# pentalpha/sickle

Hardware: AMD Instinct MI355X
Metric: reads/sec trimmed (+ Gbases/sec), 150 bp SE Sanger q20 l20, inputs resident in HBM (higher is better)
Workload: dtype u8; 1 GPU; sickle se, 10000000 synthetic 150 bp Sanger reads per GPU, q=20 l=20 (BASELINE configs[1]); mode=resident, reads_per_gpu=10000000, reads_in_job=10000000, read_len=150, stride=152, kernel=sk_scan_tile_staged_kernel

## Files before the change

### sickle_amd/csrc/sk_kernels.hip

```cpp

#include "sk_kernel_common.h"

#ifndef SK_WIDE_QUIET
#define SK_WIDE_QUIET 1
#endif
#define SK_STAGE_MIN 5
#define SK_STAGE_MAX 20
#ifndef SK_CUT_STORE_AUX
#define SK_CUT_STORE_AUX 16
#endif


template <bool UNIFORM, bool HAS_SEQ, bool MFMA, int NBUF, int ABLATE, int SEG, int STAGE, bool RAG, bool SORT = false, int WIDE = 0, int WSTAGE = 0>
__device__ __forceinline__ void
sk_scan_tile_body(const uint8_t *__restrict__ qual, const uint8_t *__restrict__ seq,
                  const uint32_t *__restrict__ lengths, sk_cut_dev *__restrict__ out,
                  unsigned long long *errword, const sk_scan_args &a, const sk_tile_dev *__restrict__ tiles,
                  const uint32_t *__restrict__ out_index, const uint64_t *__restrict__ offsets)
{
    static_assert(!SORT || (RAG && !UNIFORM && MFMA), "regrouped ragged batches: re-strided tiles, matrix path");
    static_assert(!WIDE || (RAG && UNIFORM && MFMA && !SORT), "medium reads: uniform batches, re-strided tiles, matrix path");
    static_assert(!WSTAGE || (WIDE && !HAS_SEQ), "the medium-read tiles' register stage: without -n");
    constexpr uint32_t ROWS = WIDE == 2 ? 16u : WIDE ? 32u : 64u;
    constexpr int RSHIFT = WIDE == 2 ? 4 : WIDE ? 5 : 6;
    static_assert(!RAG || (NBUF == 1 && !SEG && STAGE == 0 && ABLATE == 0), "re-strided tiles: one buffer, LDS-DMA");
    static_assert(!MFMA || UNIFORM || RAG, "the matrix path needs one window width per tile");
    constexpr bool MIXED = MFMA && !UNIFORM;
    static_assert(STAGE == 0 || (UNIFORM && !HAS_SEQ && NBUF == 1 && (SEG == 0 || SEG == 2)), "register staging: uniform tiles, one buffer");
    static_assert(!SEG || (UNIFORM && MFMA && NBUF == 1), "segmented batches run the uniform matrix path, one buffer");
    constexpr int LDS_BUFS = NBUF;
    constexpr bool SEQ_SHARES = HAS_SEQ && NBUF == 1;
    extern __shared__ __attribute__((aligned(16))) uint8_t lds[];
    const int lane = threadIdx.x & 63;
    const int rlane = WIDE == 2 ? (lane & 15) : WIDE ? (lane & 31) : lane;
    const int part = WIDE == 2 ? (lane >> 4) & 1 : 0;
    const int wave = __builtin_amdgcn_readfirstlane((int)(threadIdx.x >> 6));
    const int waves_per_block = blockDim.x >> 6;
    const uint32_t stride = a.stride;
    const uint32_t buf_bytes = (RAG || SEG) ? a.buf_bytes : 64u * stride + SK_TILE_SLACK;
    uint8_t *buf0 = lds + (size_t)wave * LDS_BUFS * buf_bytes;
    uint8_t *buf1 = LDS_BUFS > 1 ? buf0 + buf_bytes : buf0;

    const uint32_t xcd = SORT ? blockIdx.x & 7u : 0u;
    const unsigned long long *const slist = reinterpret_cast<const unsigned long long *>(tiles) + (size_t)xcd * a.n_tiles * 4u;
    const uint64_t *const perm = reinterpret_cast<const uint64_t *>(out_index) + (size_t)xcd * a.n_tiles * 64u;
    const uint64_t n_tiles = SORT ? (uint64_t)min(scalar_load(lengths + xcd), a.n_tiles) : SEG ? (uint64_t)a.n_tiles : (a.n_reads + ROWS - 1) >> RSHIFT;
    uint64_t wave_global = SORT ? (uint64_t)(blockIdx.x >> 3) : (uint64_t)blockIdx.x * waves_per_block + wave;
    const uint64_t wave_count = SORT ? (uint64_t)((gridDim.x - xcd + 7u) >> 3) : (uint64_t)gridDim.x * waves_per_block;
    if (a.tile_order == 1 && (wave_count & 7) == 0) {
        const uint64_t per = wave_count >> 3;
        wave_global = (wave_global & 7) * per + (wave_global >> 3);
    }

    const uint32_t min4 = splat((uint32_t)a.qmin), max4 = splat((uint32_t)a.qmax);
    const uint32_t hi4 = splat((uint32_t)(127 - a.qmax));
    const uint32_t cthr4 = splat((uint32_t)a.cthr);
    const int range = a.qmax - a.qmin;

    int Lu = 0, wu = 0;
    bool scan_u = false, three_blocks = false;
    sk_v4i bandA0 = {0, 0, 0, 0}, bandA1 = {0, 0, 0, 0}, bandA2 = {0, 0, 0, 0};
    sk_v16i negT;
    const int half = lane >> 5;
    constexpr bool TABLE = SEG != 0 || SORT;
    struct band3 {
        sk_v4i b0, b1, b2;
    };
    band3 band_next{{0, 0, 0, 0}, {0, 0, 0, 0}, {0, 0, 0, 0}};
    auto band_fetch = [&](int w) -> band3 {
        typedef const __attribute__((address_space(1))) sk_v4i *gv4;
        gv4 tb = (gv4)(uintptr_t)a.band_table + ((uint32_t)w * 3u * 64u + (uint32_t)lane);
        band3 b;
        b.b0 = tb[0];
        b.b1 = tb[64];
        b.b2 = (SEG == 2) ? b.b1 : tb[128];
        return b;
    };
    auto width_of = [](int len) -> int { return len / 10 ? len / 10 : len; };
    auto set_scalars = [&](int len) {
        const int w_old = wu;
        Lu = len;
        scan_u = Lu > 0 && Lu >= a.lthr;
        wu = width_of(Lu);
        three_blocks = MFMA && STAGE == 0 && (SEG == 2 ? false : SEG == 3 ? true : wu > 33);
        if (MFMA && (!TABLE || wu != w_old)) {
            const int T = a.craw * wu;
#pragma unroll
            for (int i = 0; i < 16; ++i) {
                int seed = -T;
                asm volatile("" : "+v"(seed));
                negT[i] = seed;
            }
        }
    };
    auto install_band = [&](const band3 &b) {
        bandA0 = b.b0;
        bandA1 = b.b1;
        bandA2 = b.b2;
    };
    auto set_length = [&](int len) {
        set_scalars(len);
        if (MFMA) {
            int ln = lane;
            if (MIXED) asm volatile("" : "+v"(ln));
            const int k0 = (ln >> 5) * 16;
            const int far = WIDE ? 32 * (wu / 32) : 32;
#pragma unroll
            for (int j = 0; j < 4; ++j) {
                bandA0[j] = (int)sk_band_dword(ln, wu, k0 + 4 * j);
                bandA1[j] = (int)sk_band_dword(ln, wu, k0 + 4 * j + far);
                bandA2[j] = (int)sk_band_dword(ln, wu, k0 + 4 * j + far + 32);
            }
        }
    };
    constexpr bool WRITE_THROUGH = STAGE != 0 && SEG == 0 && ABLATE != 3;
    if (!TABLE) set_length((int)a.read_len);

    const uint64_t batch_end = RAG ? rag_batch_end(offsets, lengths, a) : 0;
    auto fetch_desc = [&](uint64_t tt) -> sk_tile_dev {
        uint32_t at = (uint32_t)tt * (uint32_t)sizeof(sk_tile_dev);
        asm volatile("" : "+v"(at));
        return *reinterpret_cast<const sk_tile_dev *>(reinterpret_cast<const uint8_t *>(tiles) + at);
    };
    auto uniform_desc = [&](const sk_tile_dev &d) -> sk_tile_dev {
        sk_tile_dev u;
        u.byte_off = ((uint64_t)(uint32_t)__builtin_amdgcn_readfirstlane((int)(uint32_t)(d.byte_off >> 32)) << 32) |
                     (uint32_t)__builtin_amdgcn_readfirstlane((int)(uint32_t)d.byte_off);
        u.slot0 = (uint32_t)__builtin_amdgcn_readfirstlane((int)d.slot0);
        u.stride = (uint32_t)__builtin_amdgcn_readfirstlane((int)d.stride);
        const uint32_t rl = (uint32_t)__builtin_amdgcn_readfirstlane((int)((uint32_t)d.rows | ((uint32_t)d.read_len << 16)));
        u.rows = (uint16_t)rl;
        u.read_len = (uint16_t)(rl >> 16);
        u.reserved = 0;
        return u;
    };
    auto probe = [&](uint64_t tt, const sk_tile_dev *ahead = nullptr) -> sk_tile_view {
        sk_tile_view v;
        v.take = true;
        v.uni = false;
        v.rowoff = 0;
        if (SEG) {
            const sk_tile_dev d = ahead ? uniform_desc(*ahead) : tiles[tt];
            v.off = d.byte_off;
            v.ts = d.stride;
            v.rows = d.rows;
            v.bytes = v.rows * v.ts;
            v.len = (int)d.read_len;
            v.r = d.slot0;
        } else if (RAG && UNIFORM) {
            v.off = (tt << RSHIFT) * stride;
            v.rows = (uint32_t)min((uint64_t)ROWS, a.n_reads - (tt << RSHIFT));
            v.ts = rag_pitch<true>(a.read_len);
            v.bytes = (v.rows - 1u) * stride + a.read_len;
            v.len = (int)a.read_len;
            v.r = (tt << RSHIFT) + rlane;
        } else if (SORT) {
        } else if (RAG) {
            const sk_rag_tile g = rag_probe(tt, lane, offsets, lengths, a);
            v.off = g.start;
            v.bytes = g.span;
            v.rows = (uint32_t)min((uint64_t)64, a.n_reads - (tt << 6));
            v.ts = rag_pitch<false>((uint32_t)g.lmax);
            v.len = g.len;
            v.rowoff = g.rowoff;
            v.r = (tt << 6) + lane;
            v.take = rag_tile_fits(g, buf_bytes);
            v.uni = v.rows == 64u && __builtin_amdgcn_ballot_w64(g.len != g.lmax) == 0;
        } else {
            v.off = (tt << 6) * stride;
            v.rows = (uint32_t)min((uint64_t)64, a.n_reads - (tt << 6));
            v.ts = stride;
            v.bytes = v.rows * stride;
            v.r = (tt << 6) + lane;
            v.len = UNIFORM ? (int)a.read_len : (v.r < a.n_reads ? (int)min(lengths[v.r], stride) : 0);
        }
        return v;
    };

    struct sort_raw {
        sk_v4u d0, d1;
        uint64_t e;
    };
    auto sort_issue = [&](uint64_t tt) -> sort_raw {
        sort_raw q;
        uint32_t at = (uint32_t)tt * 32u;
        asm volatile("" : "+v"(at));
        const uint8_t *dp = reinterpret_cast<const uint8_t *>(slist) + at;
        q.d0 = *reinterpret_cast<const sk_v4u *>(dp);
        q.d1 = *reinterpret_cast<const sk_v4u *>(dp + 16);
        q.e = perm[tt * 64u + (uint32_t)lane];
        return q;
    };
    auto first = [](uint32_t x) -> uint32_t { return (uint32_t)__builtin_amdgcn_readfirstlane((int)x); };
    int sort_lmax = 0, sort_lmin = 0, sort_w = 0;
    int next_lmax = 0, next_lmin = 0, next_w = 0;
    auto sort_finish = [&](const sort_raw &q) -> sk_tile_view {
        sk_tile_view v;
        const uint32_t d00 = first(q.d0[0]), d01 = first(q.d0[1]), d02 = first(q.d0[2]), d03 = first(q.d0[3]);
        const uint32_t d10 = first(q.d1[0]), d11 = first(q.d1[1]), d12 = first(q.d1[2]);
        const uint64_t widx = d00;
        v.rows = (d01 >> 16) & 0xffu;
        next_w = (int)(d01 >> 24);
        next_lmax = (int)(d12 & 0xffffu);
        next_lmin = (int)(d12 >> 16);
        v.off = ((uint64_t)d03 << 32) | d02;
        v.bytes = d11 ? 0xffffffffu : d10;
        v.rowoff = (uint32_t)lane < v.rows ? (uint32_t)q.e : 0u;
        v.len = (uint32_t)lane < v.rows ? (int)((uint32_t)(q.e >> 32) & 0xffffu) : 0;
        v.r = widx * SK_SORT_WINDOW + (uint32_t)(q.e >> 48);
        v.ts = rag_pitch<false>((uint32_t)next_lmax);
        v.take = true;
        v.uni = true;
        return v;
    };

    auto probe_index = [&](sk_tile_view &v) { v.r = (uint64_t)((uint32_t)v.r + min((uint32_t)lane, v.rows - 1u)); };
    const bool scatter = SEG && !a.slot_order;
    auto index_issue = [&](uint64_t slot) -> uint32_t {
        uint32_t idx;
        const uint32_t *src = out_index + slot;
        asm volatile("global_load_dword %0, %1, off" : "=v"(idx) : "v"(src) : "memory");
        return idx;
    };
    auto index_settle = [&](uint32_t &idx) { asm volatile("s_waitcnt vmcnt(0)" : "+v"(idx)::"memory"); };

    typedef uint32_t sk_v4u_a4 __attribute__((ext_vector_type(4), aligned(1)));
    constexpr int WOFF = WIDE ? (WSTAGE ? WSTAGE : 32) : 0;
    uint32_t wso[WOFF ? WOFF : 1];
    sk_v4u wst[WSTAGE ? WSTAGE : 1];
    const uint32_t wpieces = WIDE ? (ROWS * (rag_pitch<true>(a.read_len) / 16u) + 63u) >> 6 : 0u;
    if (WIDE) {
        const uint32_t cpr = rag_pitch<true>(a.read_len) / 16u, qd = 64u / cpr, rd = 64u % cpr;
        const uint32_t lim = (ROWS - 1u) * stride + a.read_len - 1u;
        uint32_t rr = (uint32_t)lane / cpr, cc = (uint32_t)lane % cpr;
#pragma unroll
        for (int p = 0; p < WOFF; ++p) {
            wso[p] = min(__umul24(rr, stride) + 16u * cc, lim);
            cc += rd;
            rr += qd;
            if (cc >= cpr) {
                cc -= cpr;
                ++rr;
            }
        }
    }

    auto rag_dma = [&](const uint8_t *base, uint8_t *dst, const sk_tile_view &v) {
        constexpr uint32_t GRAN = 16u;
        const uint32_t cpr = v.ts / GRAN;
        const uint32_t qd = 64u / cpr, rd = 64u % cpr;
        uint32_t rr = (uint32_t)lane / cpr, cc = (uint32_t)lane % cpr;
        const uint8_t *src = base + v.off;
        const uint32_t lim = (v.bytes ? v.bytes : 1u) - 1u;
// ... 1 lines not shown
        if (WIDE && !WSTAGE && all_safe && v.rows == ROWS && wpieces <= (uint32_t)WOFF) {
#pragma unroll
            for (int p = 0; p < WOFF; ++p)
                if ((uint32_t)p < wpieces) dma_piece<true, false>(src + wso[p], dst + (uint32_t)p * (64u * GRAN));
            return;
        }
        auto piece = [&](uint32_t p, uint32_t ro, uint32_t cc_p) {
            const uint32_t so = min(ro + GRAN * cc_p, lim);
            const bool inside = all_safe || v.off + so + GRAN <= batch_end;
            if (__builtin_expect(all_safe || __builtin_amdgcn_ballot_w64(!inside) == 0, 1)) {
                dma_piece<true, SORT>(src + so, dst + p * (64u * GRAN));
            } else {
                if (inside) {
                    dma_piece<true, SORT>(src + so, dst + p * (64u * GRAN));
                } else {
                    for (uint32_t j = 0; j < GRAN && v.off + so + j < batch_end; ++j)
                        dst[p * (64u * GRAN) + (uint32_t)lane * GRAN + j] = src[so + j];
                }
            }
        };
        auto advance = [&]() {
            cc += rd;
            rr += qd;
            if (cc >= cpr) {
                cc -= cpr;
                ++rr;
            }
        };
        if (SORT) {
            for (uint32_t p = 0; p < cpr; p += 4) {
                uint32_t ro[4], cq[4];
#pragma unroll
                for (int u = 0; u < 4; ++u) {
                    ro[u] = (uint32_t)__builtin_amdgcn_ds_bpermute((int)(min(rr, 63u) << 2), (int)v.rowoff);
                    cq[u] = cc;
                    advance();
                }
#pragma unroll
                for (int u = 0; u < 4; ++u)
                    if (p + (uint32_t)u < cpr) piece(p + (uint32_t)u, ro[u], cq[u]);
            }
        } else {
            const uint32_t pieces = WIDE == 2 ? (cpr + 3u) >> 2 : WIDE ? (cpr + 1u) >> 1 : cpr;
            for (uint32_t p = 0; p < pieces; ++p) {
                uint32_t ro;
                if (UNIFORM) ro = WIDE ? __umul24(rr, stride) : rr * stride;
                else if (v.uni) ro = rr * (uint32_t)__builtin_amdgcn_readfirstlane(v.len);
                else ro = (uint32_t)__builtin_amdgcn_ds_bpermute((int)(rr << 2), (int)v.rowoff);
                piece(p, ro, cc);
                advance();
            }
        }
    };
    auto load_tile = [&](const uint8_t *base, uint8_t *dst, const sk_tile_view &v) {
        if (RAG) rag_dma(base, dst, v);
        else tile_to_lds(base + v.off, dst, v.bytes, lane);
    };

    auto wstage_ok = [&](const sk_tile_view &v) -> bool { return WSTAGE && v.rows == ROWS && v.off + (uint64_t)v.bytes + 16u <= batch_end; };
    auto wstage_load = [&](const sk_tile_view &v) {
        const uint8_t *src = qual + v.off;
#pragma unroll
        for (int p = 0; p < WSTAGE; ++p) wst[p] = __builtin_nontemporal_load(reinterpret_cast<const sk_v4u_a4 *>(src + wso[p]));
    };
    auto wstage_write = [&]() {
#pragma unroll
        for (int p = 0; p < WSTAGE; ++p)
            if ((uint32_t)p < wpieces) *reinterpret_cast<sk_v4u *>(buf0 + (uint32_t)p * 1024u + (uint32_t)lane * 16u) = wst[p];
    };
    bool w_cur = false, w_nxt = false;

    sk_v4u stage[STAGE ? STAGE : 1];
    const uint32_t full_bytes = 64u * stride;
    auto stage_off = [&](int p, uint32_t bytes) -> uint32_t {
        const uint32_t off = (uint32_t)p * 1024u + (uint32_t)lane * 16u;
        return (SEG || p == STAGE - 1) ? min(off, bytes - 16u) : off;
    };

    const uint64_t SEG_CHUNK = SORT ? 1ull : 1ull << a.seg_chunk_shift;
    auto next_tile = [&](uint64_t tt) -> uint64_t {
        if (SEG || SORT) return ((tt + 1) & (SEG_CHUNK - 1)) != 0 ? tt + 1 : tt + 1 + (wave_count - 1) * SEG_CHUNK;
        return tt + wave_count;
    };
    uint64_t t = (SEG || SORT) ? wave_global * SEG_CHUNK : wave_global;
    if (t >= n_tiles) return;

    sk_tile_view cur = SORT ? sort_finish(sort_issue(t)) : probe(t), nxt = cur;
    if (TABLE) band_next = band_fetch(SORT ? next_w : width_of(cur.len));
    sort_raw raw{{0, 0, 0, 0}, {0, 0, 0, 0}, 0};
    if (SEG) probe_index(cur);
    bool cur_staged = STAGE && cur.rows == 64u;
    if (cur_staged) {
        const uint32_t cb = SEG ? cur.bytes : full_bytes;
#pragma unroll
        for (int p = 0; p < STAGE; ++p)
            stage[p] = __builtin_nontemporal_load(reinterpret_cast<const sk_v4u *>(qual + cur.off + stage_off(p, cb)));
    } else if (wstage_ok(cur)) {
        wstage_load(cur);
        w_cur = true;
    } else if (cur.take) {
        load_tile(qual, buf0, cur);
    }
    if (HAS_SEQ && !SEQ_SHARES) tile_to_lds(seq + cur.off, buf1, cur.bytes, lane);
    int parity = 0;
    constexpr bool PROBE_EARLY = NBUF == 2 || STAGE != 0 || ABLATE != 0 || SEG != 0;

    sk_tile_dev ahead{};
    if (SEG) ahead = fetch_desc(min(next_tile(t), n_tiles - 1));
    for (; t < n_tiles; t = next_tile(t)) {
        const uint64_t tn = next_tile(t);
        const bool more = tn < n_tiles;
        if (PROBE_EARLY && more) nxt = probe(tn, SEG ? &ahead : nullptr);
        const uint32_t ts = cur.ts;
        const uint64_t r = cur.r;
        const uint32_t cur_bytes = cur.bytes;
        if (SEG && cur.len != Lu) {
            if (width_of(cur.len) != wu) install_band(band_next);
            set_scalars(cur.len);
        }
        const uint32_t next_bytes = (PROBE_EARLY && more) ? nxt.bytes : 0u;
        const int next_pieces = (PROBE_EARLY && more) ? tile_pieces(next_bytes) : 0;
        const uint8_t *tile;

        const bool active = (uint32_t)rlane < cur.rows;
        const int Lv = UNIFORM ? 0 : cur.len;
        bool tile_u = false;
        if (MIXED && SORT) {
            sort_lmax = next_lmax;
            sort_lmin = next_lmin;
            sort_w = next_w;
            tile_u = sort_w > 0;
            if (tile_u && sort_w != wu) {
                install_band(band_next);
                set_scalars(sort_lmax);
            }
        } else if (MIXED) {
            const int l0 = __builtin_amdgcn_readfirstlane(cur.len);
            tile_u = cur.uni && l0 > 0 && l0 / 10 <= 65;
            if (tile_u && l0 != Lu) set_length(l0);
        }

        if (SORT) {
            tile = buf0;
            wait_vmcnt(0);
            if (more) raw = sort_issue(tn);
        } else if (SEQ_SHARES || RAG) {
            tile = buf0;
            if (WSTAGE && w_cur) wstage_write();
            else wait_vmcnt(0);
        } else if (HAS_SEQ) {
            tile = buf0;
            wait_vmcnt(tile_pieces(cur_bytes));
        } else if (STAGE) {
            tile = buf0;
            const bool next_staged = more && nxt.rows == 64u && ABLATE != 2;
            if (SEG) {
                if (cur_staged && next_staged) {
                    const uint8_t *nsrc = qual + nxt.off;
#pragma unroll
                    for (int p = 0; p < STAGE; ++p) {
                        *reinterpret_cast<sk_v4u *>(buf0 + stage_off(p, cur_bytes)) = stage[p];
                        stage[p] = __builtin_nontemporal_load(reinterpret_cast<const sk_v4u *>(nsrc + stage_off(p, next_bytes)));
                    }
                } else {
                    if (cur_staged) {
#pragma unroll
                        for (int p = 0; p < STAGE; ++p) *reinterpret_cast<sk_v4u *>(buf0 + stage_off(p, cur_bytes)) = stage[p];
                    } else {
                        wait_vmcnt(0);
                    }
                    if (next_staged) {
                        const uint8_t *nsrc = qual + nxt.off;
#pragma unroll
                        for (int p = 0; p < STAGE; ++p)
                            stage[p] = __builtin_nontemporal_load(reinterpret_cast<const sk_v4u *>(nsrc + stage_off(p, next_bytes)));
                    }
                }
            } else if (cur_staged && (ABLATE != 2 || t == wave_global)) {
                const uint8_t *nsrc = qual + (next_staged ? nxt.off : cur.off);
                const uint32_t keep = next_staged ? ~0u : 1023u;
#pragma unroll
                for (int p = 0; p < STAGE; ++p) {
                    const uint32_t off = stage_off(p, full_bytes);
                    *reinterpret_cast<sk_v4u *>(buf0 + off) = stage[p];
                    stage[p] = __builtin_nontemporal_load(reinterpret_cast<const sk_v4u *>(nsrc + (off & keep)));
                }
            } else if (!cur_staged) {
                wait_vmcnt(0);
            }
            cur_staged = next_staged;
        } else if (NBUF == 1 || ABLATE == 2) {
            tile = buf0;
            wait_vmcnt(0);
        } else {
            tile = parity ? buf1 : buf0;
            uint8_t *other = parity ? buf0 : buf1;
            if (more) tile_to_lds(qual + nxt.off, other, next_bytes, lane);
            wait_vmcnt(next_pieces);
            parity ^= 1;
        }
        if (!PROBE_EARLY && !SORT && more) nxt = probe(tn);
        if (WSTAGE) {
            w_nxt = more && wstage_ok(nxt);
            if (w_nxt) wstage_load(nxt);
        }
        if (SEG) ahead = fetch_desc(min(next_tile(tn), n_tiles - 1));
        if (SEG && more) probe_index(nxt);
        if (SEG && more && width_of(nxt.len) != wu) band_next = band_fetch(width_of(nxt.len));
        uint32_t oidx = 0;
        if (scatter) oidx = index_issue(r);
        if (RAG && !cur.take) {
            if (lane == 0) {
                atomicMax(errword + 1, (unsigned long long)a.scan_id);
                atomicMax(errword + 6, (unsigned long long)(a.scan_id & 0xffffffffull) << 32);
                atomicAdd(errword + 6, 1ull);
            }
            if (more && nxt.take) load_tile(qual, buf0, nxt);
            cur = nxt;
            continue;
        }
        const uint32_t *row = reinterpret_cast<const uint32_t *>(tile + (size_t)rlane * ts);
        if (ABLATE == 1) {
            const sk_cut_dev dummy{(int)row[0], (int)row[1]};
            asm volatile("s_waitcnt lgkmcnt(0)" ::: "memory");
            if (NBUF == 1 && more && (!STAGE || !cur_staged)) tile_to_lds(qual + nxt.off, buf0, next_bytes, lane);
            if (active) out[r] = dummy;
            cur = nxt;
            continue;
        }

        const bool scanned = UNIFORM ? (active && scan_u) : (active && Lv > 0 && Lv >= a.lthr);
        const int L = UNIFORM ? (scan_u ? Lu : 0) : (scanned ? Lv : 0);
        int w = L / 10;
        if (w == 0) w = L;
        const int nwin = (UNIFORM ? scan_u : scanned) ? L - w + 1 : 0;
// ... 281 lines not shown
                const sk_v2u s5 = __builtin_amdgcn_permlane32_swap(h5, h5, false, false), s3 = __builtin_amdgcn_permlane32_swap(h3, h3, false, false);
                h5 = min(s5[0], s5[1]);
                h3 = min(s3[0], s3[1]);
                if (WIDE == 2) {
                    h5 = min(h5, (uint32_t)__builtin_amdgcn_ds_bpermute((lane ^ 16) << 2, (int)h5));
                    h3 = min(h3, (uint32_t)__builtin_amdgcn_ds_bpermute((lane ^ 16) << 2, (int)h3));
                }
            }
            if (have5 && h5 != NONE) five = 4 * k5 + (int)(h5 >> 3);
            if (done && h3 != NONE) three = 4 * k3 + (int)(h3 >> 3);
        }

        if (__builtin_amdgcn_ballot_w64(bad)) {
            if (bad) {
                const int touched = done ? i1 + w : L;
                int p = INF;
                for (int k = 0; 4 * k < L; ++k) {
                    uint32_t f = keep_first(bad_flags(row[k], min4, hi4), L - 4 * k);
                    if (f) { p = 4 * k + (__builtin_ctz(f) >> 3); break; }
                }
                if (p < touched) report_error(errword, SEG ? (uint64_t)out_index[r] : r, p, (int)(int8_t)(tile[(size_t)rlane * ts + p]));
            }
        }

        if (HAS_SEQ) {
            asm volatile("s_waitcnt lgkmcnt(0)" ::: "memory");
            if (SEQ_SHARES) {
                load_tile(seq, buf0, cur);
                wait_vmcnt(0);
                if (scatter) index_settle(oidx);
            } else {
                if (more) tile_to_lds(qual + nxt.off, buf0, next_bytes, lane);
                wait_vmcnt(next_pieces);
            }
            const uint32_t *srow = reinterpret_cast<const uint32_t *>((SEQ_SHARES ? buf0 : buf1) + (size_t)rlane * ts);
            uint32_t nlo = NONE, anyN = 0;
            auto n_step = [&](uint32_t x, uint32_t rel) {
                const uint32_t y = (x | 0x20202020u) ^ 0x6e6e6e6eu;
                const uint32_t either = ~(((y & 0x7f7f7f7fu) + 0x7f7f7f7fu) | y) & H4;
                const uint32_t lower = either & (x << 2);
                nlo = min(nlo, __builtin_elementwise_add_sat(ffbl_or_none(lower), rel));
                anyN |= either ^ lower;
            };
            {
                int k = 0;
                if (UNIFORM || tile_u) {
                    const int full = (SORT ? min(Lfull, Lmax) : Lmax) >> 2;
                    const uint64_t *srow64 = reinterpret_cast<const uint64_t *>(srow);
                    constexpr int SHARE = WIDE == 2 ? 4 : WIDE ? 2 : 1;
                    for (k = 8 * (WIDE == 2 ? lane >> 4 : WIDE ? half : 0); k + 8 <= full; k += 8 * SHARE) {
                        uint64_t x[4];
#pragma unroll
                        for (int u = 0; u < 4; ++u) x[u] = srow64[(k >> 1) + u];
#pragma unroll
                        for (int u = 0; u < 4; ++u) {
                            n_step((uint32_t)x[u], 32u * (uint32_t)(k + 2 * u));
                            n_step((uint32_t)(x[u] >> 32), 32u * (uint32_t)(k + 2 * u + 1));
                        }
                    }
                    if (WIDE) k = full & ~7;
                }
                for (; 4 * k < Lmax; ++k) n_step(first_bytes(srow[k], L - 4 * k, 0u), 32u * (uint32_t)k);
                if (WIDE) {
                    const sk_v2u sn = __builtin_amdgcn_permlane32_swap(nlo, nlo, false, false), sa = __builtin_amdgcn_permlane32_swap(anyN, anyN, false, false);
                    nlo = min(sn[0], sn[1]);
                    anyN = sa[0] | sa[1];
                    if (WIDE == 2) {
                        nlo = min(nlo, (uint32_t)__builtin_amdgcn_ds_bpermute((lane ^ 16) << 2, (int)nlo));
                        anyN |= (uint32_t)__builtin_amdgcn_ds_bpermute((lane ^ 16) << 2, (int)anyN);
                    }
                }
            }
            if (nlo != NONE) three = (int)(nlo >> 3) - 1;
            else if (anyN) three = -2;
            asm volatile("s_waitcnt lgkmcnt(0)" ::: "memory");
            if (SORT && more) {
                nxt = sort_finish(raw);
                if (next_w != wu && next_w != 0) band_next = band_fetch(next_w);
            }
            if (more) {
                if (SEQ_SHARES) { if (nxt.take) load_tile(qual, buf0, nxt); }
                else tile_to_lds(seq + nxt.off, buf1, next_bytes, lane);
            }
        } else if (NBUF == 1 && ABLATE != 2 && (!STAGE || (more && !cur_staged))) {
            asm volatile("s_waitcnt lgkmcnt(0)" ::: "memory");
            if (scatter) index_settle(oidx);
            if (SORT && more) {
                nxt = sort_finish(raw);
                if (next_w != wu && next_w != 0) band_next = band_fetch(next_w);
            }
            if (more && nxt.take && !(WSTAGE && w_nxt)) load_tile(qual, buf0, nxt);
        }
        if (WSTAGE) w_cur = w_nxt;
#if SK_TAIL_PRIO
        __builtin_amdgcn_s_setprio(0);
#endif

        if (!scanned || !found5 || (three - five < a.lthr)) {
            five = -1;
            three = -1;
        }
        if (STAGE && scatter) index_settle(oidx);
        if constexpr (WRITE_THROUGH) {
            typedef int sk_v2i __attribute__((ext_vector_type(2)));
            const __amdgpu_buffer_rsrc_t cuts = __builtin_amdgcn_make_buffer_rsrc(out + (t << 6), 0, (int)(cur.rows * 8u), 0x00020000);
            if (active) __builtin_amdgcn_raw_buffer_store_b64(sk_v2i{five, three}, cuts, lane * 8, 0, SK_CUT_STORE_AUX);
        } else if (active && (!WIDE || lane < (int)ROWS)) {
            out[scatter ? (uint64_t)oidx : r] = sk_cut_dev{five, three};
        }
        asm volatile("s_waitcnt lgkmcnt(0)" ::: "memory");
        cur = nxt;
    }
}

template <bool UNIFORM, bool HAS_SEQ, bool MFMA = false, int NBUF = 2, int ABLATE = 0, int SEG = 0>
__global__ void __launch_bounds__(SK_TILE_THREADS, 2)
sk_scan_tile_kernel(const uint8_t *__restrict__ qual, const uint8_t *__restrict__ seq,
                    const uint32_t *__restrict__ lengths, sk_cut_dev *__restrict__ out,
                    unsigned long long *errword, sk_scan_args a, const sk_tile_dev *__restrict__ tiles = nullptr,
                    const uint32_t *__restrict__ out_index = nullptr)
{
    sk_scan_tile_body<UNIFORM, HAS_SEQ, MFMA, NBUF, ABLATE, SEG, 0, false>(qual, seq, lengths, out, errword, a, tiles, out_index, nullptr);
}

template <bool UNIFORM, bool HAS_SEQ, bool MFMA>
__global__ void __launch_bounds__(SK_TILE_THREADS, 2)
sk_scan_tile_any_kernel(const uint8_t *__restrict__ qual, const uint8_t *__restrict__ seq,
                        const uint64_t *__restrict__ offsets, const uint32_t *__restrict__ lengths,
                        sk_cut_dev *__restrict__ out, unsigned long long *errword, sk_scan_args a)
{
    if (!UNIFORM && a.sort_flags && scalar_load(a.sort_flags) != 0 && scalar_load(a.sort_flags + 1) == 0) return;
    if (!UNIFORM) {
        a.n_reads = sk_counted_reads(a.n_reads_dev, a.n_reads);
        if (a.n_reads == 0) return;
    }
    sk_scan_tile_body<UNIFORM, HAS_SEQ, MFMA, 1, 0, false, 0, true>(qual, seq, lengths, out, errword, a, nullptr, nullptr, offsets);
}

template <bool HAS_SEQ>
__global__ void __launch_bounds__(SK_TILE_THREADS, 2)
sk_scan_tile_sorted_kernel(const uint8_t *__restrict__ qual, const uint8_t *__restrict__ seq,
                           const uint64_t *__restrict__ offsets, const uint64_t *__restrict__ perm,
                           const unsigned long long *__restrict__ lists, const uint32_t *__restrict__ counts,
                           sk_cut_dev *__restrict__ out, unsigned long long *errword, sk_scan_args a)
{
    if (scalar_load(a.sort_flags) == 0 || scalar_load(a.sort_flags + 1) != 0) return;
    a.n_reads = sk_counted_reads(a.n_reads_dev, a.n_reads);
    if (a.n_reads == 0) return;
    sk_scan_tile_body<false, HAS_SEQ, true, 1, 0, false, 0, true, true>(qual, seq, counts, out, errword, a, reinterpret_cast<const sk_tile_dev *>(lists),
                                                                         reinterpret_cast<const uint32_t *>(perm), offsets);
}

template <bool HAS_SEQ, int WIDE, int WSTAGE = 0>
__global__ void __launch_bounds__(SK_TILE_THREADS, 2)
sk_scan_tile_wide_kernel(const uint8_t *__restrict__ qual, const uint8_t *__restrict__ seq, sk_cut_dev *__restrict__ out,
                         unsigned long long *errword, sk_scan_args a)
{
    sk_scan_tile_body<true, HAS_SEQ, true, 1, 0, false, 0, true, false, WIDE, WSTAGE>(qual, seq, nullptr, out, errword, a, nullptr, nullptr, nullptr);
}

template <int STAGE, int ABLATE = 0>
__global__ void __launch_bounds__(64) __attribute__((amdgpu_waves_per_eu(STAGE > 10 ? 2 : 3, STAGE > 10 ? 3 : 4)))
sk_scan_tile_staged_kernel(const uint8_t *__restrict__ qual, const uint8_t *__restrict__ seq,
                           const uint32_t *__restrict__ lengths, sk_cut_dev *__restrict__ out,
                           unsigned long long *errword, sk_scan_args a, const sk_tile_dev *__restrict__ tiles = nullptr,
                           const uint32_t *__restrict__ out_index = nullptr)
{
    sk_scan_tile_body<true, false, true, 1, ABLATE, false, STAGE, false>(qual, seq, lengths, out, errword, a, tiles, out_index, nullptr);
}

template <int STAGE>
__global__ void __launch_bounds__(64) __attribute__((amdgpu_waves_per_eu(STAGE > 10 ? 2 : 3, STAGE > 10 ? 2 : 3)))
sk_scan_seg_staged_kernel(const uint8_t *__restrict__ qual, const uint8_t *__restrict__ seq,
                          const uint32_t *__restrict__ lengths, sk_cut_dev *__restrict__ out,
                          unsigned long long *errword, sk_scan_args a, const sk_tile_dev *__restrict__ tiles,
                          const uint32_t *__restrict__ out_index)
{
    sk_scan_tile_body<true, false, true, 1, 0, 2, STAGE, false>(qual, seq, lengths, out, errword, a, tiles, out_index, nullptr);
}

namespace {

int tile_nbuf_default()
{
    static const int v = [] {
        const char *e = getenv("SK_TILE_NBUF");
        return (e && (*e == '1' || *e == '2')) ? *e - '0' : SK_TILE_NBUF_DEFAULT;
    }();
    return v;
}

int tile_stage_default()
{
    static const int v = [] {
        const char *e = getenv("SK_TILE_STAGE");
        return (e && *e == '0') ? 0 : 1;
    }();
    return v;
}

template <typename K>
hipError_t launch_tile_kernel(K kern, int bufs, const uint8_t *qual, const uint8_t *seq, const uint32_t *lengths,
                              sk_cut_dev *out, unsigned long long *errword, const sk_scan_args *a, int cu_count,
                              int per_cu_cap, hipStream_t stream, bool by_registers = false)
{
    const uint32_t lds_bytes = (uint32_t)bufs * (64u * a->stride + SK_TILE_SLACK);
    if (lds_bytes > SK_LDS_PER_CU) return hipErrorInvalidValue;
    int per_cu = (int)(SK_LDS_PER_CU / lds_bytes);
    if (per_cu > 16) per_cu = 16;
    const kernel_facts facts = prepare_kernel(kern);
    if (facts.status != hipSuccess) return facts.status;
    {
        const int fits = reg_fit(facts);
        if (by_registers && getenv("SK_DEBUG_LAUNCH")) fprintf(stderr, "[sk] staged kernel: %d registers -> %d workgroups per CU\n", facts.regs, fits);
        if (per_cu > fits) per_cu = fits;
    }
    if (per_cu_cap > 0 && per_cu > per_cu_cap) per_cu = per_cu_cap;
    const uint64_t n_tiles = (a->n_reads + 63) >> 6;
    uint64_t grid = (uint64_t)cu_count * per_cu;
    if (grid > n_tiles) grid = n_tiles;
    if (grid == 0) return hipSuccess;
    hipLaunchKernelGGL(kern, dim3((unsigned)grid), dim3(64), lds_bytes, stream, qual, seq, lengths, out, errword, *a,
                       (const sk_tile_dev *)nullptr, (const uint32_t *)nullptr);
    return hipGetLastError();
}

}

extern "C" __attribute__((visibility("hidden"))) int sk_tile_is_staged(uint32_t stride, uint32_t read_len, int has_seq)
{
    const uint32_t wu = read_len / 10 ? read_len / 10 : read_len;
    const uint32_t pieces = (64u * stride + 1023u) >> 10;
    return !has_seq && read_len > 0 && wu <= 65 && tile_nbuf_default() == 1 && tile_stage_default() && stride >= 16 &&
           stride % 8 == 0 && pieces >= SK_STAGE_MIN && pieces <= SK_STAGE_MAX;
}

extern "C" __attribute__((visibility("hidden"))) hipError_t sk_launch_tile(const uint8_t *qual, const uint8_t *seq, const uint32_t *lengths,
                                     sk_cut_dev *out, unsigned long long *errword, const sk_scan_args *a,
                                     int cu_count, hipStream_t stream)
{
    const bool uniform = lengths == nullptr;
    const bool has_seq = a->truncn != 0;
    const uint32_t wu = a->read_len / 10 ? a->read_len / 10 : a->read_len;
    const bool mfma = uniform && wu <= 65 && a->read_len > 0;
    const int nbuf = tile_nbuf_default();
#define SK_GO(KERN, BUFS) launch_tile_kernel(KERN, BUFS, qual, seq, lengths, out, errword, a, cu_count, 0, stream)
    if (has_seq && nbuf == 1) {
        if (mfma) return SK_GO((sk_scan_tile_kernel<true, true, true, 1>), 1);
        if (uniform) return SK_GO((sk_scan_tile_kernel<true, true, false, 1>), 1);
        return SK_GO((sk_scan_tile_kernel<false, true, false, 1>), 1);
    }
    if (has_seq) {
        if (mfma) return SK_GO((sk_scan_tile_kernel<true, true, true, 2>), 2);
        if (uniform) return SK_GO((sk_scan_tile_kernel<true, true, false, 2>), 2);
        return SK_GO((sk_scan_tile_kernel<false, true, false, 2>), 2);
    }
    if (nbuf == 1) {
        const uint32_t pieces = (64u * a->stride + 1023u) >> 10;
        if (mfma && sk_tile_is_staged(a->stride, a->read_len, 0)) {
#define SK_STAGED(P) case P: return launch_tile_kernel(sk_scan_tile_staged_kernel<P>, 1, qual, seq, lengths, out, errword, a, cu_count, 0, stream, true)
            switch (pieces) {
                SK_STAGED(5); SK_STAGED(6); SK_STAGED(7); SK_STAGED(8); SK_STAGED(9); SK_STAGED(10);
                SK_STAGED(11); SK_STAGED(12); SK_STAGED(13); SK_STAGED(14); SK_STAGED(15); SK_STAGED(16);
                SK_STAGED(17); SK_STAGED(18); SK_STAGED(19); SK_STAGED(20);
            default: break;
            }
#undef SK_STAGED
        }
        if (mfma) return SK_GO((sk_scan_tile_kernel<true, false, true, 1>), 1);
        if (uniform) return SK_GO((sk_scan_tile_kernel<true, false, false, 1>), 1);
        return SK_GO((sk_scan_tile_kernel<false, false, false, 1>), 1);
    }
    if (mfma) return SK_GO((sk_scan_tile_kernel<true, false, true, 2>), 2);
    if (uniform) return SK_GO((sk_scan_tile_kernel<true, false, false, 2>), 2);
    return SK_GO((sk_scan_tile_kernel<false, false, false, 2>), 2);
#undef SK_GO
}

extern "C" __attribute__((visibility("hidden"))) hipError_t sk_launch_seg(const uint8_t *qual, const uint8_t *seq, const sk_tile_dev *tiles,
                                    const uint32_t *out_index, sk_cut_dev *out, unsigned long long *errword,
                                    const sk_scan_args *a, const sk_seg_class *classes, uint32_t n_classes,
                                    int cu_count, hipStream_t stream)
{
    const sk_seg_class whole = {0u, a->n_tiles, a->stride, 1u};
    if (!classes || n_classes == 0) {
        classes = &whole;
        n_classes = 1;
    }
    for (uint32_t c = 0; c < n_classes; ++c) {
        const sk_seg_class &k = classes[c];
        if (k.n_tiles == 0) continue;
        if ((uint64_t)k.first_tile + k.n_tiles > a->n_tiles || k.max_stride == 0 || k.max_stride % 8 != 0) return hipErrorInvalidValue;
        const uint32_t lds_bytes = 64u * k.max_stride + SK_TILE_SLACK;
        if (lds_bytes > SK_LDS_PER_CU) return hipErrorInvalidValue;
        int per_cu = (int)(SK_LDS_PER_CU / lds_bytes);
        if (per_cu > 16) per_cu = 16;
        uint64_t grid = (uint64_t)cu_count * per_cu;
        const uint64_t chunk = 1ull << a->seg_chunk_shift;
        const uint64_t chunks = ((uint64_t)k.n_tiles + chunk - 1) / chunk;
        if (grid > chunks) grid = chunks;
        sk_scan_args as = *a;
        as.buf_bytes = lds_bytes;
        as.n_tiles = k.n_tiles;
        auto launch = [&](auto kern, int wg_per_cu = 0) {
            const kernel_facts facts = prepare_kernel(kern);
            if (facts.status != hipSuccess) return facts.status;
            uint64_t g = grid;
            const int fit = wg_per_cu > 0 ? std::min(wg_per_cu, reg_fit(facts)) : reg_fit(facts);
            if (fit < per_cu) {
                g = (uint64_t)cu_count * fit;
                if (g > chunks) g = chunks;
            }
            hipLaunchKernelGGL(kern, dim3((unsigned)g), dim3(64), lds_bytes, stream, qual, seq,
                               (const uint32_t *)nullptr, out, errword, as, tiles + k.first_tile, out_index);
            return hipGetLastError();
        };
        hipError_t e;
        static const bool seg_stage = [] { const char *v = getenv("SK_SEG_STAGE"); return v && *v == '1'; }();
        if (seg_stage && !a->truncn && !k.wide && k.max_stride <= 320u)
            e = k.max_stride <= 160u ? launch(sk_scan_seg_staged_kernel<10>, 12) : launch(sk_scan_seg_staged_kernel<20>, 8);
        else if (a->truncn) e = k.wide ? launch(sk_scan_tile_kernel<true, true, true, 1, 0, 3>) : launch(sk_scan_tile_kernel<true, true, true, 1, 0, 2>);
        else e = k.wide ? launch(sk_scan_tile_kernel<true, false, true, 1, 0, 3>) : launch(sk_scan_tile_kernel<true, false, true, 1, 0, 2>);
        if (e != hipSuccess) return e;
    }
    return hipSuccess;
}

extern "C" __attribute__((visibility("hidden"))) hipError_t sk_launch_any(const uint8_t *qual, const uint8_t *seq, const uint64_t *offsets,
                                    const uint32_t *lengths, sk_cut_dev *out, unsigned long long *errword,
                                    const sk_scan_args *a, int cu_count, hipStream_t stream)
{
    const bool uniform = offsets == nullptr && lengths == nullptr;
    const uint32_t lds_bytes = a->buf_bytes;
    if (lds_bytes == 0 || lds_bytes > SK_LDS_PER_CU) return hipErrorInvalidValue;
    int per_cu = (int)(SK_LDS_PER_CU / lds_bytes);
    if (per_cu > 16) per_cu = 16;
    const uint64_t n_tiles = (a->n_reads + 63) >> 6;
    uint64_t grid = (uint64_t)cu_count * per_cu;
    if (grid > n_tiles) grid = n_tiles;
    if (grid == 0) return hipSuccess;
    auto launch = [&](auto kern) {
        const kernel_facts facts = prepare_kernel(kern);
        if (facts.status != hipSuccess) return facts.status;
// ... 33 lines not shown
    static const bool on = [] { const char *e = getenv("SK_WIDE_STAGE"); return !(e && *e == '0'); }();
    const uint32_t pieces = (wide_image_bytes(rows, a->read_len) - SK_TILE_SLACK) >> 10;
    (void)qual;
    return on && !a->truncn && pieces <= SK_WIDE_STAGE;
}

extern "C" __attribute__((visibility("hidden"))) uint32_t sk_wide_lds_bytes(uint32_t read_len)
{
    if (read_len / 10u < 32u || read_len > 8192u) return 0;
    const uint32_t bytes = wide_image_bytes(wide_rows(read_len), read_len);
    return bytes <= SK_LDS_PER_CU / 2u ? bytes : 0u;
}

extern "C" __attribute__((visibility("hidden"))) hipError_t sk_launch_wide(const uint8_t *qual, const uint8_t *seq, sk_cut_dev *out, unsigned long long *errword,
                                     const sk_scan_args *a, int cu_count, hipStream_t stream)
{
    sk_scan_args aw = *a;
    if (sk_wide_lds_bytes(a->read_len) == 0) return hipErrorInvalidValue;
    static const uint32_t forced_rows = [] { const char *e = getenv("SK_WIDE_ROWS"); return e ? (uint32_t)atoi(e) : 0u; }();
    static const bool stage32_on = [] { const char *e = getenv("SK_WIDE_STAGE32"); return !(e && *e == '0'); }();
    const bool staged32 = stage32_on && forced_rows != 16u && wide_staged(qual, a, 32u);
    const bool staged = !staged32 && forced_rows != 32u && wide_staged(qual, a, 16u) && (forced_rows == 16u || wide_image_bytes(32u, a->read_len) * 7u > SK_LDS_PER_CU);
    const uint32_t rows = staged32 ? 32u : staged ? 16u : wide_rows(a->read_len);
    aw.buf_bytes = wide_image_bytes(rows, a->read_len);
    int per_cu = (int)(SK_LDS_PER_CU / aw.buf_bytes);
    if (per_cu > 16) per_cu = 16;
    const uint64_t n_tiles = (a->n_reads + rows - 1) / rows;
    uint64_t grid = (uint64_t)cu_count * per_cu;
    if (grid > n_tiles) grid = n_tiles;
    if (grid == 0) return hipSuccess;
    auto launch = [&](auto kern) {
        const kernel_facts facts = prepare_kernel(kern);
        if (facts.status != hipSuccess) return facts.status;
        uint64_t g = (uint64_t)cu_count * std::min(per_cu, reg_fit(facts));
        if (g > n_tiles) g = n_tiles;
        hipLaunchKernelGGL(kern, dim3((unsigned)g), dim3(64), aw.buf_bytes, stream, qual, seq, out, errword, aw);
        return hipGetLastError();
    };
    if (staged32) return launch(sk_scan_tile_wide_kernel<false, 1, SK_WIDE_STAGE>);
    if (staged) return launch(sk_scan_tile_wide_kernel<false, 2, SK_WIDE_STAGE>);
    if (rows == 32) return a->truncn ? launch(sk_scan_tile_wide_kernel<true, 1>) : launch(sk_scan_tile_wide_kernel<false, 1>);
    return a->truncn ? launch(sk_scan_tile_wide_kernel<true, 2>) : launch(sk_scan_tile_wide_kernel<false, 2>);
}

extern "C" __attribute__((visibility("hidden"))) hipError_t sk_launch_sorted(const uint8_t *qual, const uint8_t *seq, const uint64_t *offsets, const uint64_t *perm,
                                       const unsigned long long *lists, const uint32_t *counts, sk_cut_dev *out,
                                       unsigned long long *errword, const sk_scan_args *a, int cu_count, hipStream_t stream)
{
    const uint32_t lds_bytes = a->buf_bytes;
    if (lds_bytes == 0 || lds_bytes > SK_LDS_PER_CU) return hipErrorInvalidValue;
    int per_cu = (int)(SK_LDS_PER_CU / lds_bytes);
    if (per_cu > 16) per_cu = 16;
    uint64_t grid = ((uint64_t)cu_count * per_cu) & ~7ull;
    const uint64_t most = ((a->n_reads + 63) >> 6) + 8;
    if (grid > most) grid = (most + 7) & ~7ull;
    if (grid < 8) grid = 8;
    auto launch = [&](auto kern) {
        const kernel_facts facts = prepare_kernel(kern);
        if (facts.status != hipSuccess) return facts.status;
        uint64_t g = ((uint64_t)cu_count * std::min(per_cu, reg_fit(facts))) & ~7ull;
        if (g > grid) g = grid;
        if (g < 8) g = 8;
        hipLaunchKernelGGL(kern, dim3((unsigned)g), dim3(64), lds_bytes, stream, qual, seq, offsets, perm, lists, counts, out, errword, *a);
        return hipGetLastError();
    };
    return a->truncn ? launch(sk_scan_tile_sorted_kernel<true>) : launch(sk_scan_tile_sorted_kernel<false>);
}

extern "C" hipError_t sk_launch_tile_ablate(int mode, const uint8_t *qual, sk_cut_dev *out, unsigned long long *errword,
                                            const sk_scan_args *a, int cu_count, int waves, int per_cu, hipStream_t stream)
{
    (void)waves;
#define SK_GO(KERN, BUFS) launch_tile_kernel(KERN, BUFS, qual, nullptr, nullptr, out, errword, a, cu_count, per_cu, stream)
    switch (mode) {
    case 0: return SK_GO((sk_scan_tile_kernel<true, false, true, 2, 0>), 2);
    case 1: return SK_GO((sk_scan_tile_kernel<true, false, true, 2, 1>), 2);
    case 2: return SK_GO((sk_scan_tile_kernel<true, false, true, 2, 2>), 2);
    case 10: return SK_GO((sk_scan_tile_kernel<true, false, false, 2, 0>), 2);
    case 12: return SK_GO((sk_scan_tile_kernel<true, false, false, 2, 2>), 2);
    case 100: return SK_GO((sk_scan_tile_kernel<true, false, true, 1, 0>), 1);
    case 101: return SK_GO((sk_scan_tile_kernel<true, false, true, 1, 1>), 1);
    case 102: return SK_GO((sk_scan_tile_kernel<true, false, true, 1, 2>), 1);
    case 110: return SK_GO((sk_scan_tile_kernel<true, false, false, 1, 0>), 1);
    case 200: return SK_GO((sk_scan_tile_staged_kernel<10, 0>), 1);
    case 201: return SK_GO((sk_scan_tile_staged_kernel<10, 1>), 1);
    case 202: return SK_GO((sk_scan_tile_staged_kernel<10, 2>), 1);
    case 203: return SK_GO((sk_scan_tile_staged_kernel<10, 3>), 1);
    default: return hipErrorInvalidValue;
    }
#undef SK_GO
}
```

Measured before the change: 34.68 billion reads/s.

## Split staged kernel into full-tile waves and one ragged-tail workgroup

The staged register kernel now sends the partial final tile to a dedicated last workgroup running the unstaged path. The remaining waves process only full 64-read tiles, so they can assume 64 rows, always stage the next tile in registers, and skip the per-tile fallback branch to LDS-DMA loads. This is meant to remove partial-tile checks and keep the register prefetch pipeline running without interruption. In exchange it adds a tile_first/tile_count/wave offset interface, a grid-size adjustment, new ablation modes, and a debug print.

```diff
diff --git a/sickle_amd/csrc/sk_kernels.hip b/sickle_amd/csrc/sk_kernels.hip
--- a/sickle_amd/csrc/sk_kernels.hip
+++ b/sickle_amd/csrc/sk_kernels.hip
@@ -16,8 +16,11 @@
 sk_scan_tile_body(const uint8_t *__restrict__ qual, const uint8_t *__restrict__ seq,
                   const uint32_t *__restrict__ lengths, sk_cut_dev *__restrict__ out,
                   unsigned long long *errword, const sk_scan_args &a, const sk_tile_dev *__restrict__ tiles,
-                  const uint32_t *__restrict__ out_index, const uint64_t *__restrict__ offsets)
-{
+                  const uint32_t *__restrict__ out_index, const uint64_t *__restrict__ offsets,
+                  const uint64_t tile_first = 0, const uint64_t tile_count = ~0ull, const uint64_t wave_limit = 0,
+                  const uint64_t wave_first = 0)
+{
+    constexpr bool FULL = STAGE != 0 && SEG == 0 && (ABLATE == 0 || ABLATE == 3 || ABLATE == 5);
     static_assert(!SORT || (RAG && !UNIFORM && MFMA), "regrouped ragged batches: re-strided tiles, matrix path");
     static_assert(!WIDE || (RAG && UNIFORM && MFMA && !SORT), "medium reads: uniform batches, re-strided tiles, matrix path");
     static_assert(!WSTAGE || (WIDE && !HAS_SEQ), "the medium-read tiles' register stage: without -n");
@@ -44,9 +47,10 @@
     const uint32_t xcd = SORT ? blockIdx.x & 7u : 0u;
     const unsigned long long *const slist = reinterpret_cast<const unsigned long long *>(tiles) + (size_t)xcd * a.n_tiles * 4u;
     const uint64_t *const perm = reinterpret_cast<const uint64_t *>(out_index) + (size_t)xcd * a.n_tiles * 64u;
-    const uint64_t n_tiles = SORT ? (uint64_t)min(scalar_load(lengths + xcd), a.n_tiles) : SEG ? (uint64_t)a.n_tiles : (a.n_reads + ROWS - 1) >> RSHIFT;
-    uint64_t wave_global = SORT ? (uint64_t)(blockIdx.x >> 3) : (uint64_t)blockIdx.x * waves_per_block + wave;
-    const uint64_t wave_count = SORT ? (uint64_t)((gridDim.x - xcd + 7u) >> 3) : (uint64_t)gridDim.x * waves_per_block;
+    const uint64_t n_tiles = SORT ? (uint64_t)min(scalar_load(lengths + xcd), a.n_tiles) : SEG ? (uint64_t)a.n_tiles :
+                             tile_count != ~0ull ? tile_first + tile_count : (a.n_reads + ROWS - 1) >> RSHIFT;
+    uint64_t wave_global = SORT ? (uint64_t)(blockIdx.x >> 3) : (uint64_t)blockIdx.x * waves_per_block + wave - wave_first;
+    const uint64_t wave_count = SORT ? (uint64_t)((gridDim.x - xcd + 7u) >> 3) : wave_limit ? wave_limit : (uint64_t)gridDim.x * waves_per_block;
     if (a.tile_order == 1 && (wave_count & 7) == 0) {
         const uint64_t per = wave_count >> 3;
         wave_global = (wave_global & 7) * per + (wave_global >> 3);
@@ -168,7 +172,7 @@
             v.uni = v.rows == 64u && __builtin_amdgcn_ballot_w64(g.len != g.lmax) == 0;
         } else {
             v.off = (tt << 6) * stride;
-            v.rows = (uint32_t)min((uint64_t)64, a.n_reads - (tt << 6));
+            v.rows = FULL ? 64u : (uint32_t)min((uint64_t)64, a.n_reads - (tt << 6));
             v.ts = stride;
             v.bytes = v.rows * stride;
             v.r = (tt << 6) + lane;
@@ -336,19 +340,21 @@
         if (SEG || SORT) return ((tt + 1) & (SEG_CHUNK - 1)) != 0 ? tt + 1 : tt + 1 + (wave_count - 1) * SEG_CHUNK;
         return tt + wave_count;
     };
-    uint64_t t = (SEG || SORT) ? wave_global * SEG_CHUNK : wave_global;
+    uint64_t t = (SEG || SORT) ? wave_global * SEG_CHUNK : wave_global + tile_first;
     if (t >= n_tiles) return;
 
     sk_tile_view cur = SORT ? sort_finish(sort_issue(t)) : probe(t), nxt = cur;
     if (TABLE) band_next = band_fetch(SORT ? next_w : width_of(cur.len));
     sort_raw raw{{0, 0, 0, 0}, {0, 0, 0, 0}, 0};
     if (SEG) probe_index(cur);
-    bool cur_staged = STAGE && cur.rows == 64u;
+    bool cur_staged = STAGE && (FULL || cur.rows == 64u);
     if (cur_staged) {
         const uint32_t cb = SEG ? cur.bytes : full_bytes;
 #pragma unroll
-        for (int p = 0; p < STAGE; ++p)
+        for (int p = 0; p < STAGE; ++p) {
             stage[p] = __builtin_nontemporal_load(reinterpret_cast<const sk_v4u *>(qual + cur.off + stage_off(p, cb)));
+            if (FULL && ABLATE == 5) __builtin_amdgcn_sched_barrier(0);
+        }
     } else if (wstage_ok(cur)) {
         wstage_load(cur);
         w_cur = true;
@@ -405,6 +411,17 @@
         } else if (HAS_SEQ) {
             tile = buf0;
             wait_vmcnt(tile_pieces(cur_bytes));
+        } else if (FULL) {
+            tile = buf0;
+            const uint8_t *nsrc = qual + (more ? nxt.off : cur.off);
+            const uint32_t keep = more ? ~0u : 1023u;
+            if (ABLATE != 5) wait_vmcnt_imm<0>();
+#pragma unroll
+            for (int p = 0; p < STAGE; ++p) {
+                const uint32_t off = stage_off(p, full_bytes);
+                *reinterpret_cast<sk_v4u *>(buf0 + off) = stage[p];
+                stage[p] = __builtin_nontemporal_load(reinterpret_cast<const sk_v4u *>(nsrc + (off & keep)));
+            }
         } else if (STAGE) {
             tile = buf0;
             const bool next_staged = more && nxt.rows == 64u && ABLATE != 2;
@@ -852,7 +869,7 @@
                 if (SEQ_SHARES) { if (nxt.take) load_tile(qual, buf0, nxt); }
                 else tile_to_lds(seq + nxt.off, buf1, next_bytes, lane);
             }
-        } else if (NBUF == 1 && ABLATE != 2 && (!STAGE || (more && !cur_staged))) {
+        } else if (NBUF == 1 && ABLATE != 2 && !FULL && (!STAGE || (more && !cur_staged))) {
             asm volatile("s_waitcnt lgkmcnt(0)" ::: "memory");
             if (scatter) index_settle(oidx);
             if (SORT && more) {
@@ -936,7 +953,19 @@
                            unsigned long long *errword, sk_scan_args a, const sk_tile_dev *__restrict__ tiles = nullptr,
                            const uint32_t *__restrict__ out_index = nullptr)
 {
-    sk_scan_tile_body<true, false, true, 1, ABLATE, false, STAGE, false>(qual, seq, lengths, out, errword, a, tiles, out_index, nullptr);
+    if constexpr (ABLATE == 0 || ABLATE == 3 || ABLATE == 5) {
+        const uint64_t full = a.n_reads >> 6;
+        const uint32_t ragged = (a.n_reads & 63u) != 0 ? 1u : 0u;
+        if (ragged && blockIdx.x == gridDim.x - 1u) {
+            sk_scan_tile_body<true, false, true, 1, 0, false, 0, false>(qual, seq, lengths, out, errword, a, tiles, out_index, nullptr,
+                                                                        full, 1, 1, gridDim.x - 1u);
+            return;
+        }
+        sk_scan_tile_body<true, false, true, 1, ABLATE, false, STAGE, false>(qual, seq, lengths, out, errword, a, tiles, out_index, nullptr,
+                                                                             0, full, gridDim.x - ragged);
+    } else {
+        sk_scan_tile_body<true, false, true, 1, ABLATE, false, STAGE, false>(qual, seq, lengths, out, errword, a, tiles, out_index, nullptr);
+    }
 }
 
 template <int STAGE>
@@ -972,7 +1001,7 @@
 template <typename K>
 hipError_t launch_tile_kernel(K kern, int bufs, const uint8_t *qual, const uint8_t *seq, const uint32_t *lengths,
                               sk_cut_dev *out, unsigned long long *errword, const sk_scan_args *a, int cu_count,
-                              int per_cu_cap, hipStream_t stream, bool by_registers = false)
+                              int per_cu_cap, hipStream_t stream, bool by_registers = false, bool full_tiles = false)
 {
     const uint32_t lds_bytes = (uint32_t)bufs * (64u * a->stride + SK_TILE_SLACK);
     if (lds_bytes > SK_LDS_PER_CU) return hipErrorInvalidValue;
@@ -988,8 +1017,16 @@
     if (per_cu_cap > 0 && per_cu > per_cu_cap) per_cu = per_cu_cap;
     const uint64_t n_tiles = (a->n_reads + 63) >> 6;
     uint64_t grid = (uint64_t)cu_count * per_cu;
-    if (grid > n_tiles) grid = n_tiles;
+    if (full_tiles) {
+        const uint64_t extra = (a->n_reads & 63u) ? 1u : 0u, n_full = a->n_reads >> 6;
+        const uint64_t room = grid > extra ? grid - extra : 1u;
+        grid = (n_full < room ? n_full : room) + extra;
+    } else if (grid > n_tiles) {
+        grid = n_tiles;
+    }
     if (grid == 0) return hipSuccess;
+    if (by_registers && getenv("SK_DEBUG_LAUNCH"))
+        fprintf(stderr, "[sk] staged kernel: %d workgroups per CU on %d CUs, grid %llu\n", per_cu, cu_count, (unsigned long long)grid);
     hipLaunchKernelGGL(kern, dim3((unsigned)grid), dim3(64), lds_bytes, stream, qual, seq, lengths, out, errword, *a,
                        (const sk_tile_dev *)nullptr, (const uint32_t *)nullptr);
     return hipGetLastError();
@@ -1028,7 +1065,7 @@
     if (nbuf == 1) {
         const uint32_t pieces = (64u * a->stride + 1023u) >> 10;
         if (mfma && sk_tile_is_staged(a->stride, a->read_len, 0)) {
-#define SK_STAGED(P) case P: return launch_tile_kernel(sk_scan_tile_staged_kernel<P>, 1, qual, seq, lengths, out, errword, a, cu_count, 0, stream, true)
+#define SK_STAGED(P) case P: return launch_tile_kernel(sk_scan_tile_staged_kernel<P>, 1, qual, seq, lengths, out, errword, a, cu_count, 0, stream, true, true)
             switch (pieces) {
                 SK_STAGED(5); SK_STAGED(6); SK_STAGED(7); SK_STAGED(8); SK_STAGED(9); SK_STAGED(10);
                 SK_STAGED(11); SK_STAGED(12); SK_STAGED(13); SK_STAGED(14); SK_STAGED(15); SK_STAGED(16);
@@ -1228,11 +1265,15 @@
     case 101: return SK_GO((sk_scan_tile_kernel<true, false, true, 1, 1>), 1);
     case 102: return SK_GO((sk_scan_tile_kernel<true, false, true, 1, 2>), 1);
     case 110: return SK_GO((sk_scan_tile_kernel<true, false, false, 1, 0>), 1);
-    case 200: return SK_GO((sk_scan_tile_staged_kernel<10, 0>), 1);
+#define SK_GO_FULL(KERN) launch_tile_kernel(KERN, 1, qual, nullptr, nullptr, out, errword, a, cu_count, per_cu, stream, false, true)
+    case 200: return SK_GO_FULL((sk_scan_tile_staged_kernel<10, 0>));
     case 201: return SK_GO((sk_scan_tile_staged_kernel<10, 1>), 1);
     case 202: return SK_GO((sk_scan_tile_staged_kernel<10, 2>), 1);
-    case 203: return SK_GO((sk_scan_tile_staged_kernel<10, 3>), 1);
+    case 203: return SK_GO_FULL((sk_scan_tile_staged_kernel<10, 3>));
+    case 204: return SK_GO((sk_scan_tile_staged_kernel<10, 4>), 1);
+    case 205: return SK_GO_FULL((sk_scan_tile_staged_kernel<10, 5>));
     default: return hipErrorInvalidValue;
     }
+#undef SK_GO_FULL
 #undef SK_GO
 }
```

Result: no change. 34.73 billion reads/s, median of 5 (+0.1%).
